# MeowMeowLady/InstanceSeg-Without-Voxelwise-Labeling

Hardware: AMD Instinct MI355X
Metric: voxels/sec end-to-end infer_simple (128^3 vol); 3D-conv TFLOPS vs roofline (higher is better)
Workload: dtype f32; 1 GPU; detection-mode infer_simple, host to host: pinned raw u16 volumes -> H2D -> norm1 -> dsn_body -> RPN -> proposals -> RoIAlign3D -> 2-MLP head -> decode -> NMS -> cross-tile NMS -> one all_gather of detections -> D2H; batch of 4 x (1x128^3) per rank, 3 distinct batches rotating [configs[2]]; volumes_per_rank=4

## Files before the change

include/m3d.h:

```cpp
#ifndef M3D_H_
#define M3D_H_
#include <stddef.h>
#include <stdint.h>

#ifdef __cplusplus
extern "C" {
#endif

#define M3D_OK 0
#define M3D_EINVAL (-1)
#define M3D_ELAUNCH (-2)
#define M3D_EWORKSPACE (-3)
#define M3D_EUNSUPPORTED (-4)

int m3d_version(void);
const char* m3d_error_string(int code);
const char* m3d_last_hip_error(void);
int m3d_set_option(const char* name, int value);
int m3d_get_option(const char* name, int* value);
int m3d_tuning_build(void);

int m3d_roi_align3d_forward(int aligned_slices, int aligned_height, int aligned_width, float spatial_scale,
                            int sampling_ratio, const float* d_features, int batch, int channels, int slices,
                            int height, int width, const float* d_rois, int num_rois, int roi_cols,
// ... 320 lines not shown
int m3d_conv3d_x3_pack(const float* d_weight, int cin, int cout, int relu_weights, void* d_packed, void* stream);
int m3d_conv3d_x3_forward(const float* d_x, const void* d_packed, float* d_out, int batch, int cin, int cout, int depth, int height,
                          int width, const float* d_in_offset, void* stream);
size_t m3d_conv3d_x3_workspace_bytes(int batch, int cin, int cout, int depth, int height, int width);
int m3d_conv3d_x3_forward_ws(const float* d_x, const void* d_packed, float* d_out, int batch, int cin, int cout, int depth, int height,
                             int width, const float* d_in_offset, void* d_workspace, size_t workspace_bytes, void* stream);
size_t m3d_conv3d_x3f_packed_bytes(int cin, int cout);
int m3d_conv3d_x3f_pack(const float* d_weight, int cin, int cout, int relu_weights, void* d_packed, void* stream);
int m3d_conv3d_x3f_forward_ws(const float* d_x, const void* d_packed, float* d_out, int batch, int cin, int cout, int depth, int height,
                              int width, const float* d_in_offset, const float* d_in_max, void* d_workspace, size_t workspace_bytes,
                              void* stream);
long long m3d_conv3d_x3_launch_units(int batch, int cin, int cout, int depth, int height, int width);

int m3d_conv3d_zw_supported(int cin, int cout, int depth, int height, int width, int pool);
size_t m3d_conv3d_zw_packed_bytes(int cin, int cout);
int m3d_conv3d_zw_pack(const float* d_weight, int cin, int cout, void* d_packed, void* stream);
int m3d_conv3d_zw_pack_dgrad(const float* d_weight, int cin, int cout, void* d_packed, void* stream);
int m3d_conv3d_zw_slots(void);
long long m3d_conv3d_zw_launch_units(int batch, int cin, int cout, int depth, int height, int width);
int m3d_conv3d_zw_bound_of(const float* d_x, long long n, float* d_slots, void* stream);
int m3d_conv3d_zw_forward(const float* d_in, const void* d_packed, float* d_out, int batch, int cin, int cout, int depth, int height,
                          int width, const float* d_scale, const float* d_shift, int relu, int pool, const float* d_in_max,
                          float* d_out_max, void* stream);
int m3d_conv3d_zn_supported(int cin, int cout, int depth, int height, int width);
size_t m3d_conv3d_zn_packed_bytes(int cin, int cout);
int m3d_conv3d_zn_pack(const float* d_weight, int cin, int cout, void* d_packed, void* stream);
int m3d_conv3d_zn_pack_dgrad(const float* d_weight, int cin, int cout, void* d_packed, void* stream);
long long m3d_conv3d_zn_launch_units(int batch, int cin, int cout, int depth, int height, int width);
int m3d_conv3d_zn_forward(const float* d_in, const void* d_packed, float* d_out, int batch, int cin, int cout, int depth, int height,
                          int width, const float* d_scale, const float* d_shift, int relu, const float* d_in_max, float* d_out_max,
                          void* stream);
int m3d_conv3d_zn_dilated_supported(int cin, int cout, int depth, int height, int width, int dilation);
long long m3d_conv3d_zn_dilated_launch_units(int batch, int cin, int cout, int depth, int height, int width, int dilation);
int m3d_conv3d_zn_dilated_forward(const float* d_in, const void* d_packed, float* d_out, int batch, int cin, int cout, int depth,
                                  int height, int width, int dilation, const float* d_scale, const float* d_shift, int relu,
                                  const float* d_in_max, float* d_out_max, void* stream);
int m3d_prm_strip_absmax(const float* d_strip, long long rows, int L, int pitch, int num_peaks, float* d_out, void* stream);
int m3d_conv3d_zw_forward_strip(const float* d_in, const void* d_packed, float* d_out, int cin, int cout, int depth, int height,
                                int width, const float* d_col_bound, int num_peaks, int pitch, void* stream);
int m3d_prm_strip_dgrad_prepare_zw(const float* d_gn, const void* d_packed, int cin, int cout, int num_peaks, int window, int in_slab,
                                   const int32_t* d_origin, const float* d_xnext, const float* d_norm, const float* d_scale,
                                   const float* d_up_offset, int depth, int height, int width, int out_slab,
                                   const float* d_col_bound, float* d_out, int32_t* d_origin_out, void* stream);

int m3d_prm_strip_dgrad_prepare(const float* d_gn, const float* d_packed, int cin, int cout, int num_peaks, int window, int in_slab,
                                const int32_t* d_origin, const float* d_xnext, const float* d_norm, const float* d_scale,
// ... 203 lines not shown
```

instanceseg-without-voxelwise-labeling_amd/csrc/fc_gemm.hip:

```cpp
#include <type_traits>

#include "f16x2.h"

namespace {

using namespace m3d::f16x2;

constexpr int BM = 128, BN = 128, BK = 32, LS = BK + 4;
constexpr int kStageFloats = (BM + BN) * LS;

struct FcArgs {
  const float* x; const float* w; const float* bias; float* out; float* part;
  int M, N, K, mt, nt, slices, chunks, relu;
  int slices_tail;
  int mt_full;
  int full_per_xcd, tail_per_xcd;
};

__global__ __launch_bounds__(256, 2) void fc_gemm_kernel(FcArgs a) {
  extern __shared__ float lds[];
  const int tid = threadIdx.x, lane = tid & 63, wave = tid >> 6;
  const int xcd = blockIdx.x & 7, idx = blockIdx.x >> 3;
  const int tiles_full = a.mt_full * a.nt, nfull = tiles_full * a.slices, ntail = (a.mt - a.mt_full) * a.nt * a.slices_tail;
  int slice, tile;
// ... 876 lines not shown
  }
  if (const int ts = m3d::opt(m3d::OPT_TUNE_FC_SLICES); ts > 0) bs = bt = ts < p.chunks ? ts : p.chunks;
  if (const int ts = m3d::opt(m3d::OPT_TUNE_FC_SLICES_TAIL); ts > 0) bt = ts < p.chunks ? ts : p.chunks;
  p.slices = bs; p.slices_tail = ntail_tiles ? bt : 1;
  p.full_per_xcd = (p.mt_full * p.nt * bs + 7) / 8;
  p.tail_per_xcd = (ntail_tiles * p.slices_tail + 7) / 8;
  return p;
}

X3Plan x3b_plan(int M, int N, int K) {
  X3Plan p{8, (M + 255) / 256, (N + 255) / 256, x3b_slices(M, N, K), 0};
  p.per_xcd = (p.mt * p.nt * p.slices + 7) / 8;
  return p;
}

inline bool f16x2_big_tiles(int M, int N) {
  const int w = m3d::opt(m3d::OPT_TUNE_FC_X3_ROWS);
  if (w == 128 || w == 256) return false;
  if (w == 512) return true;
  return M >= 384 && N >= 256;
}
X3Plan f16x2_plan(int M, int N, int K) { return f16x2_big_tiles(M, N) ? x3b_plan(M, N, K) : x3_plan(M, N, K); }

}

M3D_API int m3d_linear_plan(int kind, int M, int N, int K, int* tile_rows, int* tile_cols, int* slices, int* slices_tail,
                            int* full_row_tiles) {
  if (kind < 0 || kind > 3 || M <= 0 || N <= 0 || K <= 0) return M3D_EINVAL;
  if (K % (kind == 0 ? 4 : 32) != 0) return M3D_EUNSUPPORTED;
  int tr, tc, s, st, fm;
  if (kind == 0) {
    const Plan p = make_plan(M, N, K);
    tr = BM; tc = BN; s = p.slices; st = p.slices_tail; fm = p.mt_full;
  } else {
    const X3Plan p = kind == 1 ? x3_plan(M, N, K) : (kind == 2 ? x3b_plan(M, N, K) : f16x2_plan(M, N, K));
    tr = p.wr == 8 ? 256 : 64 * p.wr; tc = p.wr == 8 ? 256 : BN; s = st = p.slices; fm = p.mt;
  }
  if (tile_rows) *tile_rows = tr;
  if (tile_cols) *tile_cols = tc;
  if (slices) *slices = s;
  if (slices_tail) *slices_tail = st;
  if (full_row_tiles) *full_row_tiles = fm;
  return M3D_OK;
}

M3D_API size_t m3d_linear_workspace_bytes(int M, int N, int K) {
  if (M <= 0 || N <= 0 || K <= 0) return 0;
  const Plan p = make_plan(M, N, K);
  const int sm = p.slices > p.slices_tail ? p.slices : p.slices_tail;
  return sm > 1 ? (size_t)sm * M * N * sizeof(float) : 16;
}

M3D_API int m3d_linear_forward(const float* d_x, const float* d_weight, const float* d_bias, float* d_out, int M, int N, int K,
                               int relu, void* d_ws, size_t ws_bytes, void* stream) {
  if (M < 0 || N <= 0 || K <= 0) return M3D_EINVAL;
  if (M == 0) return M3D_OK;
  if (!d_x || !d_weight || !d_out) return M3D_EINVAL;
  if (K % 4 != 0 || ((uintptr_t)d_x & 15) || ((uintptr_t)d_weight & 15)) return M3D_EUNSUPPORTED;
  const Plan p = make_plan(M, N, K);
  const int sm = p.slices > p.slices_tail ? p.slices : p.slices_tail;
  if (sm > 1 && (!d_ws || ws_bytes < (size_t)sm * M * N * sizeof(float))) return M3D_EWORKSPACE;
  FcArgs a{d_x, d_weight, d_bias, d_out, (float*)d_ws, M, N, K, p.mt, p.nt, p.slices, p.chunks, relu, p.slices_tail, p.mt_full,
           p.full_per_xcd, p.tail_per_xcd};
  const size_t lds = sizeof(float) * 2 * kStageFloats;
  hipStream_t st = m3d::as_stream(stream);
  (void)hipFuncSetAttribute(reinterpret_cast<const void*>(fc_gemm_kernel), hipFuncAttributeMaxDynamicSharedMemorySize, (int)lds);
  hipLaunchKernelGGL(fc_gemm_kernel, dim3(8 * (p.full_per_xcd + p.tail_per_xcd)), dim3(256), lds, st, a);
  if (sm > 1) {
    const long long MN = (long long)M * N;
    long long blocks = (MN + 255) / 256;
    if (blocks > 4096) blocks = 4096;
    hipLaunchKernelGGL(fc_reduce_kernel, dim3((unsigned)blocks), dim3(256), 0, st, (const float*)d_ws, d_bias, d_out, MN, N, p.slices,
                       p.slices_tail, (long long)(p.mt_full < p.mt ? p.mt_full * BM : M) * N, relu, (unsigned*)nullptr);
  }
  return m3d::check_launch("linear_forward");
}

M3D_API size_t m3d_linear_bf16x3_packed_bytes(int N, int K) {
  if (N <= 0 || K <= 0 || K % 32 != 0) return 0;
  return (size_t)((N + BN - 1) / BN) * (K / 32) * X3_CHUNK_U4 * 16;
}
// ... 213 lines not shown
```

instanceseg-without-voxelwise-labeling_amd/m3d/_lib.py:

```python
import ctypes as C
import os

_HERE = os.path.dirname(os.path.abspath(__file__))
LIB_PATH = os.environ.get("M3D_LIB_PATH") or os.path.join(os.path.dirname(_HERE), "csrc", "libm3d.so")

M3D_OK = 0
_lib = None

SYMBOLS = [
    "m3d_version", "m3d_error_string", "m3d_last_hip_error", "m3d_set_option", "m3d_get_option", "m3d_tuning_build",
    "m3d_conv3d_stem5_prepare_dgrad_weights", "m3d_conv3d_stem5_dgrad", "m3d_norm1_workspace_bytes", "m3d_norm1", "m3d_norm1_batched", "m3d_norm1_stats",
    "m3d_linear_workspace_bytes", "m3d_linear_forward", "m3d_linear_bf16x3_packed_bytes", "m3d_linear_bf16x3_pack", "m3d_absmax", "m3d_linear_f16x2_packed_bytes", "m3d_linear_f16x2_pack", "m3d_linear_f16x2_workspace_bytes", "m3d_linear_f16x2_forward", "m3d_linear_f16x2_forward_bounds", "m3d_linear_plan",
    "m3d_box_head_workspace_bytes", "m3d_box_head_forward",
    "m3d_linear_bf16x3_workspace_bytes", "m3d_linear_bf16x3_forward", "m3d_mask_paste3d_workspace_bytes", "m3d_mask_paste3d", "m3d_linear_bf16x3_w32_workspace_bytes", "m3d_linear_bf16x3_w32_forward", "m3d_roi_align3d_tap_tables", "m3d_linear_bf16x3_roi_workspace_bytes", "m3d_linear_bf16x3_roi_forward",
    "m3d_fused_max_boxes", "m3d_compact_rows", "m3d_compact_rows2", "m3d_box_head_outputs", "m3d_conv3d_forward_split_sigmoid", "m3d_generate_proposals3d_batched_workspace_bytes", "m3d_generate_proposals3d_batched",
    "m3d_box_results3d_batched_workspace_bytes", "m3d_box_results3d_batched", "m3d_nms3d_batched_workspace_bytes", "m3d_nms3d_batched",
    "m3d_roi_align3d_forward", "m3d_roi_align3d_forward_exact", "m3d_roi_align3d_backward", "m3d_roi_align3d_workspace_bytes", "m3d_roi_align3d_forward_ws", "m3d_roi_align3d_forward_ws2", "m3d_roi_align3d_forward_ws3",
    "m3d_roi_align3d_backward_ordered_workspace_bytes", "m3d_roi_align3d_backward_ordered",
    "m3d_nms3d_workspace_bytes", "m3d_nms3d", "m3d_bbox_overlaps3d", "m3d_bbox_transform3d",
    "m3d_generate_proposals3d_workspace_bytes", "m3d_generate_proposals3d",
    "m3d_conv3d_packed_weight_bytes", "m3d_conv3d_pack_weights", "m3d_conv3d_forward", "m3d_conv3d_forward_dilated", "m3d_conv3d_forward_windowed", "m3d_conv3d_forward_pool2", "m3d_conv3d_direct_plan", "m3d_conv3d_direct_plan_count",
    "m3d_prm_seed", "m3d_prm_seed_ex", "m3d_prm_strip_geometry", "m3d_prm_prepare_plan", "m3d_prm_stem_dgrad_plan", "m3d_prm_select_peaks", "m3d_prm_select_peaks_ex", "m3d_prm_prepare", "m3d_prm_stem_prepare_weights", "m3d_prm_stem_dgrad", "m3d_prm_scatter", "m3d_prm_den_pool", "m3d_prm_stem_mfma_prepare_weights", "m3d_prm_stem_dgrad_fused_supported", "m3d_prm_stem_dgrad_fused", "m3d_prm_stem_dgrad_fused_ex", "m3d_prm_prepare_ex", "m3d_prm_stem_dgrad_fused_ex2", "m3d_prm_prepare_ex2", "m3d_prm_prepare_ex3", "m3d_prm_strip_dgrad_prepare", "m3d_conv3d_x3_packed_bytes", "m3d_conv3d_x3f_packed_bytes", "m3d_conv3d_x3f_pack", "m3d_conv3d_x3f_forward_ws", "m3d_reduce_minmax_multi", "m3d_reduce_minmax_multi_workspace_bytes", "m3d_conv3d_x3_supported", "m3d_conv3d_x3_pack", "m3d_conv3d_x3_forward", "m3d_conv3d_x3_workspace_bytes", "m3d_conv3d_x3_forward_ws", "m3d_conv3d_x3_launch_units", "m3d_conv3d_zw_supported", "m3d_conv3d_zw_packed_bytes", "m3d_conv3d_zw_pack", "m3d_conv3d_zw_slots", "m3d_conv3d_zw_launch_units", "m3d_conv3d_zw_bound_of", "m3d_conv3d_zw_forward", "m3d_conv3d_zw_forward_strip", "m3d_prm_strip_dgrad_prepare_zw", "m3d_prm_strip_absmax", "m3d_prm_small_dgrad_packed_bytes", "m3d_prm_small_dgrad_pack", "m3d_prm_small_dgrad_f16_supported", "m3d_prm_small_dgrad_f16_packed_bytes", "m3d_prm_small_dgrad_f16_pack", "m3d_prm_small_dgrad_f16_workspace_bytes", "m3d_prm_small_dgrad_f16", "m3d_prm_small_dgrad",
    "m3d_maxpool3d_2x_forward", "m3d_maxpool3d_2x_backward",
    "m3d_reduce_min_workspace_bytes", "m3d_reduce_min", "m3d_reduce_min_multi_workspace_bytes", "m3d_reduce_min_multi",
# ... 9 lines not shown
    "m3d_label_components_workspace_bytes", "m3d_label_components", "m3d_label_counts", "m3d_paint_spheres_workspace_bytes", "m3d_paint_spheres",
    "m3d_rpn_targets_workspace_bytes", "m3d_rpn_targets", "m3d_rpn_targets_wide", "m3d_rpn_loss",
    "m3d_box_head_targets_workspace_bytes", "m3d_box_head_targets", "m3d_box_head_target_blobs", "m3d_box_head_loss",
    "m3d_bn_stats", "m3d_bn_invstd", "m3d_bn_apply", "m3d_bn_backward",
    "m3d_sgd_chunk", "m3d_sgd_step", "m3d_sgd_step_scaled", "m3d_adam_step", "m3d_grad_clip_coef",
    "m3d_train_sample",
    "m3d_linear_dgrad_workspace_bytes", "m3d_linear_dgrad", "m3d_linear_wgrad_workspace_bytes", "m3d_linear_wgrad",
    "m3d_mask_targets", "m3d_mask_loss_workspace_bytes", "m3d_mask_loss",
    "m3d_conv3d_zw_pack_dgrad", "m3d_conv3d_gy_reduce",
    "m3d_peak_stimulation3d_workspace_bytes", "m3d_peak_stimulation3d", "m3d_peak_stimulation3d_backward",
    "m3d_upconv3d_2x_forward", "m3d_upconv3d_2x_dgrad_workspace_bytes", "m3d_upconv3d_2x_dgrad", "m3d_upconv3d_2x_wgrad_workspace_bytes",
    "m3d_upconv3d_2x_wgrad", "m3d_upconv3d_2x_slices",
    "m3d_conv3d_wgrad_dilated_workspace_bytes", "m3d_conv3d_wgrad_dilated", "m3d_conv3d_wgrad_dilated_tile", "m3d_conv3d_wgrad_dilated_plan",
    "m3d_conv3d_wgrad_narrow_supported", "m3d_conv3d_wgrad_narrow_workspace_bytes", "m3d_conv3d_wgrad_narrow_plan", "m3d_conv3d_wgrad_narrow",
    "m3d_conv3d_wgrad_narrow_f16x2_supported", "m3d_conv3d_wgrad_narrow_f16x2_workspace_bytes", "m3d_conv3d_wgrad_narrow_f16x2_plan",
    "m3d_conv3d_wgrad_narrow_f16x2",
    "m3d_conv3d_wgrad_narrow_dilated_f16x2_supported", "m3d_conv3d_wgrad_narrow_dilated_f16x2_workspace_bytes",
    "m3d_conv3d_wgrad_narrow_dilated_f16x2_plan", "m3d_conv3d_wgrad_narrow_dilated_f16x2",
    "m3d_conv3d_zn_supported", "m3d_conv3d_zn_packed_bytes", "m3d_conv3d_zn_pack", "m3d_conv3d_zn_pack_dgrad", "m3d_conv3d_zn_launch_units",
    "m3d_conv3d_zn_forward",
    "m3d_conv3d_zn_dilated_supported", "m3d_conv3d_zn_dilated_launch_units", "m3d_conv3d_zn_dilated_forward",
    "m3d_upconv3d_2x_f16x2_supported", "m3d_upconv3d_2x_f16x2_packed_bytes", "m3d_upconv3d_2x_f16x2_pack", "m3d_upconv3d_2x_forward_f16x2",
    "m3d_mask_tail_f16x2",
    "m3d_linear_backward_f16x2_supported", "m3d_linear_dgrad_f16x2_plan", "m3d_linear_wgrad_f16x2_plan",
    "m3d_linear_dgrad_f16x2_workspace_bytes", "m3d_linear_wgrad_f16x2_workspace_bytes", "m3d_linear_dgrad_f16x2", "m3d_linear_wgrad_f16x2",
]


class SgdTensor(C.Structure):
    _fields_ = [("p", C.c_void_p), ("g", C.c_void_p), ("m", C.c_void_p), ("n", C.c_longlong), ("lr", C.c_float), ("wd", C.c_float)]


class AdamTensor(C.Structure):
    _fields_ = [("p", C.c_void_p), ("g", C.c_void_p), ("m", C.c_void_p), ("v", C.c_void_p), ("n", C.c_longlong), ("lr_step", C.c_float),
                ("bc2_sqrt", C.c_float), ("wd", C.c_float)]


class GradTensor(C.Structure):
    _fields_ = [("g", C.c_void_p), ("n", C.c_longlong)]


class TrainImage(C.Structure):
    _fields_ = [("vol", C.c_void_p), ("stats", C.c_void_p), ("boxes", C.c_void_p), ("dtype", C.c_int), ("depth", C.c_int),
                ("height", C.c_int), ("width", C.c_int), ("num_boxes", C.c_int), ("start_max", C.c_int * 3)]


# ... 30 lines not shown
        raise M3DError("%s not built: run `python -c 'import __graft_entry__ as g; g.build()'` "
                       "or `make -C instanceseg-without-voxelwise-labeling_amd/csrc`. There is no CPU fallback." % path)
    L = C.CDLL(path)
    L.m3d_error_string.restype = C.c_char_p
    L.m3d_last_hip_error.restype = C.c_char_p
    L.m3d_conv3d_wino2_score.restype = C.c_double
    L.m3d_conv3d_wino2_local_score.restype = C.c_double
    L.m3d_prm_strip_geometry.restype = C.c_int64
    L.m3d_conv3d_x3_launch_units.restype = C.c_longlong
    L.m3d_conv3d_zw_launch_units.restype = C.c_longlong
    L.m3d_conv3d_zn_launch_units.restype = C.c_longlong
    L.m3d_conv3d_zn_dilated_launch_units.restype = C.c_longlong
    for n in ("m3d_roi_align3d_workspace_bytes", "m3d_roi_align3d_backward_ordered_workspace_bytes","m3d_nms3d_workspace_bytes", "m3d_generate_proposals3d_workspace_bytes",
              "m3d_conv3d_packed_weight_bytes", "m3d_conv3d_x3_packed_bytes", "m3d_conv3d_x3f_packed_bytes", "m3d_conv3d_zw_packed_bytes", "m3d_reduce_minmax_multi_workspace_bytes", "m3d_conv3d_x3_workspace_bytes", "m3d_reduce_min_workspace_bytes", "m3d_reduce_min_multi_workspace_bytes", "m3d_norm1_workspace_bytes", "m3d_prm_small_dgrad_packed_bytes", "m3d_prm_small_dgrad_f16_packed_bytes", "m3d_prm_small_dgrad_f16_workspace_bytes", "m3d_linear_workspace_bytes", "m3d_linear_bf16x3_packed_bytes", "m3d_linear_bf16x3_workspace_bytes", "m3d_linear_f16x2_packed_bytes", "m3d_linear_f16x2_workspace_bytes", "m3d_linear_bf16x3_w32_workspace_bytes", "m3d_linear_bf16x3_roi_workspace_bytes", "m3d_mask_paste3d_workspace_bytes", "m3d_generate_proposals3d_batched_workspace_bytes",
              "m3d_box_results3d_batched_workspace_bytes", "m3d_nms3d_batched_workspace_bytes", "m3d_otsu2d_workspace_bytes",
              "m3d_cc_workspace_bytes", "m3d_conv3d_wgrad_workspace_bytes", "m3d_conv3d_wino_packed_weight_bytes", "m3d_conv3d_wino2_packed_weight_bytes", "m3d_conv3d_wino2_workspace_bytes", "m3d_conv3d_wino2_local_workspace_bytes", "m3d_conv3d_stem_wino_packed_weight_bytes",
              "m3d_label_overlap_workspace_bytes", "m3d_box_union_overlap_workspace_bytes", "m3d_label_components_workspace_bytes",
              "m3d_paint_spheres_workspace_bytes", "m3d_rpn_targets_workspace_bytes", "m3d_box_head_targets_workspace_bytes",
              "m3d_box_head_workspace_bytes", "m3d_linear_dgrad_workspace_bytes", "m3d_linear_wgrad_workspace_bytes",
              "m3d_mask_loss_workspace_bytes", "m3d_conv3d_wgrad_f16x2_workspace_bytes", "m3d_peak_stimulation3d_workspace_bytes",
              "m3d_upconv3d_2x_dgrad_workspace_bytes", "m3d_upconv3d_2x_wgrad_workspace_bytes",
              "m3d_conv3d_wgrad_dilated_workspace_bytes", "m3d_conv3d_wgrad_narrow_workspace_bytes", "m3d_conv3d_zn_packed_bytes",
              "m3d_conv3d_wgrad_narrow_f16x2_workspace_bytes", "m3d_conv3d_wgrad_narrow_dilated_f16x2_workspace_bytes",
              "m3d_upconv3d_2x_f16x2_packed_bytes", "m3d_linear_dgrad_f16x2_workspace_bytes", "m3d_linear_wgrad_f16x2_workspace_bytes"):
        getattr(L, n).restype = C.c_size_t
    return L


def lib():
    global _lib
    if _lib is None:
        knobs = [(env, name) for env, name in _TUNE_ENV if env in os.environ]
        if knobs and "M3D_LIB_PATH" not in os.environ:
            _lib = _load(TUNE_LIB_PATH)
        else:
            _lib = _load(LIB_PATH)
        if knobs and _lib.m3d_tuning_build():
            for env, name in knobs:
                set_option(name, int(os.environ[env]))
    return _lib


class tuning:

    def __enter__(self):
        global _lib, _tune
        lib()
# ... 34 lines not shown
```

instanceseg-without-voxelwise-labeling_amd/m3d/model.py:

```python
import ctypes as C
import os

import numpy as np
import torch

from . import ops
from .conv_plan import LayerConv

BN_EPS = 1e-5


def dsn_layers(stride):
    if stride == 8:
        return [("conv1a", "bn1a", True), ("conv2a", "bn2a", False), ("conv2b", "bn2b", True), ("conv3a", "bn3a", False),
                ("conv3b", "bn3b", True), ("conv4a", "bn4a", False), ("conv4b", "bn4b", False)]
    return [("conv1a", "bn1a", True), ("conv2a", "bn2a", False), ("conv2b", "bn2b", True), ("conv3a", "bn3a", False),
            ("conv3b", "bn3b", False)]


class Probe:

    def __init__(self):
        self.spans = {}

# ... 38 lines not shown
class DetectorM3D:
    def __init__(self, params, cfg):
        self.cfg = cfg
        self.P = params
        self.probe = None
        n_head_convs = self._check_conv_head(params, cfg) if "Box_Head.convs.0.weight" in params else 0
        self.anchors = np.ascontiguousarray(cfg.anchors, dtype=np.float64)
        self.wino_mode = int(os.environ.get("M3D_WINO", "2"))
        self.use_wino = self.wino_mode != 0
        self.conv_f16 = self.use_wino and os.environ.get("M3D_CONV_F16", "1") == "1"
        self.head_conv_f16 = self.conv_f16 and os.environ.get("M3D_HEAD_CONV_F16", "0") == "1"
        self.body, self.convs = [], []
        for cname, bname, pool in dsn_layers(cfg.stride):
            c, b = "Conv_Body." + cname, "Conv_Body." + bname
            scale = (params[b + ".weight"] / torch.sqrt(params[b + ".running_var"] + BN_EPS)).contiguous()
            shift = ((params[c + ".bias"] - params[b + ".running_mean"]) * scale + params[b + ".bias"]).contiguous()
            self.convs.append(LayerConv(params[c + ".weight"], scale, shift, pool, self.wino_mode, self.conv_f16))
            self.body.append((self.convs[-1].conv, scale, shift, pool))
        self.rpn_conv_bias = params["RPN.RPN_conv.bias"].contiguous()
        self.rpn_conv = LayerConv(params["RPN.RPN_conv.weight"], None, self.rpn_conv_bias, False, self.wino_mode, self.conv_f16)
        self.A = params["RPN.RPN_cls_score.weight"].shape[0]
        w = torch.cat([params["RPN.RPN_cls_score.weight"], params["RPN.RPN_bbox_pred.weight"]], 0).contiguous()
        self.rpn_heads = ops.PackedConv3d(w)
        self.rpn_heads_bias = torch.cat([params["RPN.RPN_cls_score.bias"], params["RPN.RPN_bbox_pred.bias"]]).contiguous()
        self.conv_head = "Box_Head.convs.0.weight" in params
        self.has_head = self.conv_head or "Box_Head.fc1.weight" in params
        self.roi_gemm = os.environ.get("M3D_ROI_GEMM", "0") == "1"
        if self.has_head:
            self.outs_w = torch.cat([params["Box_Outs.cls_score.weight"], params["Box_Outs.bbox_pred.weight"]], 0).contiguous()
            self.outs_b = torch.cat([params["Box_Outs.cls_score.bias"], params["Box_Outs.bbox_pred.bias"]]).contiguous()
            self.fc_split = {}
            mode = os.environ.get("M3D_FC_SPLIT", "f16x2")
            if self.conv_head:
                self.head_convs = self._conv_head_layers(params, n_head_convs)
            if mode != "0":
                cls = ops.SplitLinear if mode in ("bf16x3", "1") else ops.SplitLinearF16
                for name in (("fc",) if self.conv_head else ("fc1", "fc2")):
                    w = params["Box_Head.%s.weight" % name]
                    if cls.supported(w):
                        self.fc_split[name] = cls(w, params["Box_Head.%s.bias" % name])

    @staticmethod
    def _check_conv_head(params, cfg):
        n = 0
        while "Box_Head.convs.%d.weight" % (2 * n) in params:
            n += 1
# ... 18 lines not shown
        kw = dict(narrow_f16=True) if self.head_conv_f16 else {}
        return [LayerConv(params["Box_Head.convs.%d.weight" % (2 * i)], None, params["Box_Head.convs.%d.bias" % (2 * i)].contiguous(), False,
                          self.wino_mode, self.conv_f16, **kw) for i in range(n)]

    def body_layer(self, li, x, bound_slot=None):
        return self.convs[li](x, self._bound, bound_slot)

    @staticmethod
    def _carried_bound(x):
        b = getattr(x, "_m3d_bound", None)
        return b[0] if b is not None and b[1] == x._version else None

    @staticmethod
    def _bound(x):
        b = DetectorM3D._carried_bound(x)
        return b if b is not None else ops.ZwConv3d.bound_of(x)

    def span(self, name):
        return self.probe(name) if self.probe is not None else _NOSPAN

    ISSUED_FRACTION = {"winograd F(2x2,3x3)": 4.0 / 9.0, "winograd F(2x4,3x3)": 1.0 / 3.0, "winograd F(2,3)x": 2.0 / 3.0,
                       "winograd F(2,5)x stem": 78.0 / 125.0, "direct": 1.0, "f16x2 F(2,3)z": 2.0}
    F16_KINDS = ("f16x2 F(2,3)z",)

    def conv_work(self, batch, size):
        out = {}
        S, H, W = size

        def record(layer):
            kind = layer.plan((batch, S, H, W)).kind
            f16 = kind in self.F16_KINDS
            pad = (layer.cout + 63) // 64 * 64 / float(layer.cout) if f16 else (layer.cout + 31) // 32 * 32 / float(layer.cout)
            alg = 2.0 * layer.cin * layer.cout * layer.k ** 3 * S * H * W * batch
            return dict(algorithmic_flop=alg, issued_flop=alg * self.ISSUED_FRACTION[kind] * pad, kernel=kind,
                        shape="%d->%d k%d @ %dx%dx%d" % (layer.cin, layer.cout, layer.k, S, H, W), dtype="f16" if f16 else "f32")
        for (cname, _, pool), layer in zip(dsn_layers(self.cfg.stride), self.convs):
            out[cname] = record(layer)
            if pool:
                S, H, W = S // 2, H // 2, W // 2
        r = record(self.rpn_conv)
        cout, nh = self.rpn_conv.cout, 7 * self.A
        alg_h = 2.0 * cout * nh * S * H * W * batch
        out["rpn"] = dict(algorithmic_flop=r["algorithmic_flop"] + alg_h, issued_flop=r["issued_flop"] + alg_h * ((nh + 31) // 32 * 32 / float(nh)),
                          dtype=r["dtype"], kernel=r["kernel"] + " (3^3 conv) + direct (the two 1^3 heads as one conv)",
                          shape="%d->%d k3, %d->%d k1 @ %dx%dx%d" % (self.rpn_conv.cin, cout, cout, nh, S, H, W))
        return out

    def conv_body(self, x, first=0, last=None):
        names = dsn_layers(self.cfg.stride)
        slots = torch.zeros((len(self.body) + 1, ops.ZwConv3d.SLOTS), dtype=torch.float32, device=x.device) if self.conv_f16 else None
        for li in range(first, len(self.body) if last is None else last):
            with self.span(names[li][0]):
                x = self.body_layer(li, x, slots[li] if slots is not None else None)
        if slots is not None:
            x._m3d_head_bound = slots[len(self.body)]
        return x

    def capture_body(self, x, first=0, last=None):
        torch.cuda.synchronize()
        side = torch.cuda.Stream()
        side.wait_stream(torch.cuda.current_stream())
        with torch.cuda.stream(side):
            for _ in range(2):
                self.conv_body(x, first, last)
        torch.cuda.current_stream().wait_stream(side)
        g = torch.cuda.CUDAGraph()
        with torch.cuda.graph(g):
            out = self.conv_body(x, first, last)
        return g.replay, out

    def rpn(self, feat):
        return self.rpn_outputs(self.rpn_conv(feat, self._bound, out_max=False))

    def rpn_outputs(self, h):
        return self.rpn_heads.split_sigmoid(h, self.A, shift=self.rpn_heads_bias)

    def _fused_ok(self, prob):
        total = prob.shape[-4] * prob.shape[-3] * prob.shape[-2] * prob.shape[-1]
        k = total if (self.cfg.pre_nms_topN <= 0 or self.cfg.pre_nms_topN >= total) else self.cfg.pre_nms_topN
        return k <= ops.fused_max_boxes()

    def proposals(self, prob, deltas, im_info, item=0):
        c = self.cfg
        if self._fused_ok(prob):
            rois, probs, kidx, num = ops.generate_proposals3d_batched(
                prob[item:item + 1], deltas[item:item + 1], self.anchors, float(c.stride), im_info, c.pre_nms_topN,
                c.post_nms_topN, c.rpn_nms_thresh, c.rpn_min_size, first_batch_index=item)
            r = int(num.item())
            return rois[0, :r], probs[0, :r].unsqueeze(1), kidx[0, :r]
        return ops.generate_proposals3d(prob[item].contiguous(), deltas[item], self.anchors, float(c.stride), im_info,
                                        c.pre_nms_topN, c.post_nms_topN, c.rpn_nms_thresh, c.rpn_min_size, batch_index=item)

    def box_head_outputs(self, feat, rois, clip_to=None):
        c, P = self.cfg, self.P
        if self.conv_head:
            return self._conv_head_outputs(feat, rois, clip_to)
        if self.probe is None and self._one_call_ok(feat, rois, int(rois.shape[0])):
# ... 277 lines not shown
```

instanceseg-without-voxelwise-labeling_amd/m3d/ops.py:

```python
import ctypes as C
import math
import threading

import numpy as np
import torch

from ._lib import lib, check, M3DError, SgdTensor, AdamTensor, GradTensor, BoxHead, TrainImage, MaskImage

BBOX_XFORM_CLIP = float(np.log(1000. / 16.))

__all__ = ["compact_rows", "compact_rows2", "box_head_outputs", "roi_align3d_forward", "roi_align3d_backward", "roi_align3d_backward_ordered", "nms3d", "bbox_overlaps3d", "bbox_transform3d",
           "generate_proposals3d", "generate_proposals3d_batched", "box_results3d_batched", "nms3d_batched", "fused_max_boxes", "PackedConv3d", "maxpool3d_2x", "maxpool3d_2x_backward", "reduce_min", "reduce_min_multi", "norm1", "norm1_batched", "norm1_stats", "train_sample", "linear", "linear_plan", "linear_dgrad", "linear_wgrad", "linear_dgrad_f16x2", "linear_wgrad_f16x2", "linear_backward_f16x2_supported", "linear_dgrad_f16x2_plan", "linear_wgrad_f16x2_plan", "upconv3d_2x_forward", "upconv3d_2x_dgrad", "upconv3d_2x_wgrad", "upconv3d_2x_slices", "UPCONV_KINDS", "UpConvF16", "SplitLinear", "linear_roi_fused", "mask_paste3d",
           "otsu2d_batch", "prm_quantize_u8", "prm_quantize_windows_u8", "prm_quantize_windows_compact_u8", "roi_normalize", "conv3d_wgrad", "conv3d_wgrad_f16x2", "conv3d_wgrad_f16x2_supported", "conv3d_wgrad_f16x2_plan", "conv3d_wgrad_narrow_f16x2", "conv3d_wgrad_narrow_f16x2_supported", "conv3d_wgrad_narrow_f16x2_plan", "conv3d_direct_plan", "conv3d_bias_grad", "conv3d_gy_reduce", "WinoConv3d", "ZwConv3d", "ZnConv3d", "X3Conv3d", "StemWinoConv3d", "gaussian_filter_u16", "median_filter3_u16", "cc_largest_batch", "binary_closing6_batch", "paint_instances", "paint_instances_into", "paint_finish", "paint_begin", "crop_offsets", "upload_packed", "conv3d_windowed", "prm_seed", "strip_geometry", "prm_prepare_plan", "prm_stem_dgrad_plan", "PRM_PREPARE_KERNELS", "PRM_STEM_DGRAD_LAYOUTS", "prm_select_peaks", "PinnedPool", "upload", "prm_prepare", "prm_stem_dgrad", "prm_stem_prepare_weights", "SmallWindowDgrad", "prm_den_pool", "prm_stem_mfma_weights", "prm_stem_dgrad_fused", "prm_stem_dgrad_fused_supported", "prm_scatter", "conv3d_stem5_dgrad", "conv3d_stem5_dgrad_weights", "label_overlap", "label_iou_best", "box_union_overlap_counts", "Overlap", "IouBest", "LABEL_LIMIT", "label_components", "label_counts", "paint_spheres", "rpn_target_sets", "rpn_target_blobs", "rpn_loss_grad", "box_head_target_sets", "box_head_target_blobs", "box_head_loss_grad", "mask_target_sets", "mask_loss_grad", "bn_stats", "bn_invstd", "bn_apply", "bn_backward", "sgd_step", "sgd_chunk", "sgd_step_scaled", "adam_step", "grad_clip_coef", "M3DError", "BBOX_XFORM_CLIP", "W_PLAIN", "W_RELU", "W_DGRAD", "W_DGRAD_RELU"]

W_PLAIN, W_RELU, W_DGRAD, W_DGRAD_RELU = 0, 1, 2, 3


def _stream():
    return C.c_void_p(torch.cuda.current_stream().cuda_stream)


def _need_gpu(*ts):
    for t in ts:
        if t is not None and not t.is_cuda:
# ... 1600 lines not shown
    def units(self, shape, dilation=1):
        if int(dilation) == 1:
            return super().units(shape)
        B = int(shape[0]) if len(shape) == 5 else 1
        D, H, W = (int(v) for v in shape[-3:])
        return int(lib().m3d_conv3d_zn_dilated_launch_units(B, self.cin, self.cout, D, H, W, int(dilation)))

    def __call__(self, x, in_max, scale=None, shift=None, relu=False, out=None, out_max=None, dilation=1):
        x, out, out_max = self._operands(x, in_max, out, out_max)
        B, cin, D, H, W = x.shape
        if int(dilation) != 1:
            check(lib().m3d_conv3d_zn_dilated_forward(_ptr(x), _ptr(self.packed), _ptr(out), B, cin, self.cout, D, H, W, int(dilation),
                                                      _ptr(scale) if scale is not None else None, _ptr(shift) if shift is not None else None,
                                                      int(bool(relu)), _ptr(in_max), _ptr(out_max) if out_max is not None else None,
                                                      _stream()), "conv3d_zn_dilated_forward")
            return out, out_max
        check(lib().m3d_conv3d_zn_forward(_ptr(x), _ptr(self.packed), _ptr(out), B, cin, self.cout, D, H, W,
                                          _ptr(scale) if scale is not None else None, _ptr(shift) if shift is not None else None,
                                          int(bool(relu)), _ptr(in_max), _ptr(out_max) if out_max is not None else None,
                                          _stream()), "conv3d_zn_forward")
        return out, out_max


class WinoConv3d(object):

    def __init__(self, weight, two_d=False, local=False):
        _need_gpu(weight)
        w = _f32c(weight)
        assert w.dim() == 5 and tuple(w.shape[2:]) == (3, 3, 3)
        self.cout, self.cin = int(w.shape[0]), int(w.shape[1])
        self.two_d = bool(two_d)
        self.local = bool(local) and self.two_d
        L = lib()
        self._bytes, self._pack, self._fwd, self._pool = \
            (L.m3d_conv3d_wino2_packed_weight_bytes, L.m3d_conv3d_wino2_pack_weights, L.m3d_conv3d_wino2_forward,
             L.m3d_conv3d_wino2_forward_pool2) if self.two_d else \
            (L.m3d_conv3d_wino_packed_weight_bytes, L.m3d_conv3d_wino_pack_weights, L.m3d_conv3d_wino_forward,
             L.m3d_conv3d_wino_forward_pool2)
        nbytes = self._bytes(self.cin, self.cout)
        self.packed = torch.empty((nbytes // 4,), dtype=torch.float32, device=w.device)
        check(self._pack(_ptr(w), self.cin, self.cout, _ptr(self.packed), _stream()), "wino_pack")

    def supports(self, width, shape=None):
        if width < (12 if self.two_d else 24):
            return False
        if self.two_d and shape is not None:
# ... 993 lines not shown
```

Before: 2.954 billion voxels/s.

## Add f16x2 MFMA pointwise RPN head kernel and small-N linear path

Adds a split-f16 MFMA 1x1x1 convolution kernel for the fused RPN cls/bbox heads, with sigmoid applied to the first split channels, and wires it behind an opt-in environment flag. It also routes linear layers with N<=32 to a new per-wave dot-product kernel instead of the tiled GEMM. The head path is meant to replace the direct FP32 pointwise conv with matrix-core work. The small-N path is meant to avoid large GEMM tiles that are mostly wasted when N is tiny. The f16 path is off by default (M3D_RPN_HEADS_F16=0), so only the small-N linear change runs by default.

After: 2.954 billion voxels/s, median of 2. No clear change (-0.0%).

```diff
diff --git a/include/m3d.h b/include/m3d.h
--- a/include/m3d.h
+++ b/include/m3d.h
@@ -366,6 +366,12 @@
 int m3d_conv3d_zw_forward(const float* d_in, const void* d_packed, float* d_out, int batch, int cin, int cout, int depth, int height,
                           int width, const float* d_scale, const float* d_shift, int relu, int pool, const float* d_in_max,
                           float* d_out_max, void* stream);
+int m3d_conv1x1_f16x2_supported(int cin, int cout);
+size_t m3d_conv1x1_f16x2_packed_bytes(int cin, int cout);
+int m3d_conv1x1_f16x2_pack(const float* d_weight, int cin, int cout, void* d_packed, void* stream);
+int m3d_conv1x1_f16x2_split_sigmoid(const float* d_in, const void* d_packed, float* d_out_sigmoid, float* d_out_rest, int batch, int cin,
+                                    int cout, int split, int depth, int height, int width, const float* d_shift, const float* d_in_max,
+                                    void* stream);
 int m3d_conv3d_zn_supported(int cin, int cout, int depth, int height, int width);
 size_t m3d_conv3d_zn_packed_bytes(int cin, int cout);
 int m3d_conv3d_zn_pack(const float* d_weight, int cin, int cout, void* d_packed, void* stream);
diff --git a/instanceseg-without-voxelwise-labeling_amd/csrc/conv1x1_f16.hip b/instanceseg-without-voxelwise-labeling_amd/csrc/conv1x1_f16.hip
--- /dev/null
+++ b/instanceseg-without-voxelwise-labeling_amd/csrc/conv1x1_f16.hip
@@ -0,0 +1,189 @@
+#include "f16x2.h"
+
+namespace {
+
+using namespace m3d::f16x2;
+
+constexpr int PW_NT = 512, PW_WAVES = 8;
+constexpr int PW_TV = 32;
+constexpr int PW_CG = 32 * PW_WAVES;
+constexpr int PW_STEP_UNITS = PW_WAVES * 128;
+constexpr int PW_PF = 4;
+constexpr int PW_MAX_CIN = 1024;
+
+__global__ __launch_bounds__(256) void pw_pack_kernel(const float* __restrict__ w, int cin, int cout, u32x4* __restrict__ packed,
+                                                      const float* __restrict__ wamax) {
+  float sw, inv;
+  f16_scale_of(*wamax, sw, inv);
+  const int steps = cin / 16, ncg = (cout + PW_CG - 1) / PW_CG;
+  const long long total = (long long)ncg * steps * PW_WAVES * 64;
+  for (long long e = (long long)blockIdx.x * 256 + threadIdx.x; e < total; e += (long long)gridDim.x * 256) {
+    const int row = (int)(e & 31), kh = (int)((e >> 5) & 1), cb = (int)((e >> 6) & (PW_WAVES - 1));
+    const long long r = e >> 9;
+    const int t = (int)(r % steps), cg = (int)(r / steps);
+    const int co = cg * PW_CG + cb * 32 + row;
+    u32x4 ph, pl;
+#pragma unroll
+    for (int j = 0; j < 4; ++j) {
+      f16x2 hh, ll;
+#pragma unroll
+      for (int u = 0; u < 2; ++u) {
+        const float v = co < cout ? w[(size_t)co * cin + t * 16 + 8 * kh + 2 * j + u] * sw : 0.f;
+        cut(v, hh, ll, u);
+      }
+      ph[j] = __builtin_bit_cast(unsigned, hh); pl[j] = __builtin_bit_cast(unsigned, ll);
+    }
+    u32x4* dst = packed + ((size_t)(cg * steps + t) * PW_WAVES + cb) * 128 + kh * 32 + row;
+    dst[0] = ph; dst[64] = pl;
+  }
+}
+
+struct PwArgs {
+  const float* x; const u32x4* wp; const float* wamax; const float* bias; const float* in_max;
+  float* out_sig; float* out_rest;
+  int cin, cout, split;
+  long long V;
+};
+
+__global__ __launch_bounds__(PW_NT, 4) void conv1x1_f16_kernel(PwArgs a) {
+  extern __shared__ float lds_f[];
+  u32x4* const lds = reinterpret_cast<u32x4*>(lds_f);
+  const int tid = threadIdx.x, lane = tid & 63;
+  const int wave = __builtin_amdgcn_readfirstlane(tid >> 6);
+  const int b = blockIdx.y, cg = blockIdx.z;
+  const long long v0 = (long long)blockIdx.x * PW_TV;
+  const int steps = a.cin / 16, kgs = a.cin / 8, plane = kgs * PW_TV;
+
+  float xs, inv_x, inv_w;
+  {
+    float sw_;
+    f16_scale_of(bound_of_slots(a.in_max, lane), xs, inv_x);
+    f16_scale_of(*a.wamax, sw_, inv_w);
+  }
+
+  const int co0 = cg * PW_CG + wave * 32;
+  const bool active = co0 < a.cout;
+  const u32x4* wq = a.wp + ((size_t)cg * steps * PW_WAVES + wave) * 128 + lane;
+  f16x8 nh[PW_PF], nl[PW_PF];
+  auto load_w = [&](int g) __attribute__((always_inline)) {
+#pragma unroll
+    for (int i = 0; i < PW_PF; ++i) {
+      const int t = min(g * PW_PF + i, steps - 1);
+      nh[i] = __builtin_bit_cast(f16x8, wq[(size_t)t * PW_STEP_UNITS]);
+      nl[i] = __builtin_bit_cast(f16x8, wq[(size_t)t * PW_STEP_UNITS + 64]);
+    }
+  };
+  if (active) load_w(0);
+
+  const float* xb = a.x + (size_t)b * a.cin * a.V;
+  for (int it0 = 0; it0 < plane; it0 += 2 * PW_NT) {
+    float v[2][8];
+    int it[2];
+#pragma unroll
+    for (int i = 0; i < 2; ++i) {
+      it[i] = it0 + i * PW_NT + tid;
+      const int itc = min(it[i], plane - 1);
+      const int kg = itc >> 5, vox = itc & 31;
+      const long long p = min(v0 + vox, a.V - 1);
+      const float* src = xb + (size_t)(8 * kg) * a.V + p;
+#pragma unroll
+      for (int j = 0; j < 8; ++j) v[i][j] = src[(size_t)j * a.V];
+    }
+#pragma unroll
+    for (int i = 0; i < 2; ++i) {
+      if (it[i] >= plane) continue;
+      u32x4 ph, pl;
+#pragma unroll
+      for (int j = 0; j < 4; ++j) {
+        f16x2 hh, ll;
+        cut(v[i][2 * j] * xs, v[i][2 * j + 1] * xs, hh, ll);
+        ph[j] = __builtin_bit_cast(unsigned, hh); pl[j] = __builtin_bit_cast(unsigned, ll);
+      }
+      lds[it[i]] = ph;
+      lds[plane + it[i]] = pl;
+    }
+  }
+  __syncthreads();
+  if (!active) return;
+
+  const int c = lane & 31, h = lane >> 5;
+  f32x16 acc[2];
+#pragma unroll
+  for (int i = 0; i < 2; ++i)
+#pragma unroll
+    for (int g = 0; g < 16; ++g) acc[i][g] = 0.f;
+  const int groups = (steps + PW_PF - 1) / PW_PF;
+  for (int g = 0; g < groups; ++g) {
+    f16x8 ch[PW_PF], cl[PW_PF];
+#pragma unroll
+    for (int i = 0; i < PW_PF; ++i) { ch[i] = nh[i]; cl[i] = nl[i]; }
+    if (g + 1 < groups) load_w(g + 1);
+#pragma unroll
+    for (int i = 0; i < PW_PF; ++i) {
+      const int t = g * PW_PF + i;
+      if (t < steps) {
+        const f16x8 bh = __builtin_bit_cast(f16x8, lds[(2 * t + h) * PW_TV + c]);
+        const f16x8 bl = __builtin_bit_cast(f16x8, lds[plane + (2 * t + h) * PW_TV + c]);
+        mfma3(ch[i], cl[i], bh, bl, acc[i & 1]);
+      }
+    }
+  }
+
+  const long long p = v0 + c;
+  if (p >= a.V) return;
+  const float un = inv_x * inv_w;
+  const int nrest = a.cout - a.split;
+#pragma unroll
+  for (int g = 0; g < 16; ++g) {
+    const int co = co0 + acc_row(g) + 4 * h;
+    if (co >= a.cout) continue;
+    float v = (acc[0][g] + acc[1][g]) * un;
+    if (a.bias) v += a.bias[co];
+    if (co < a.split) a.out_sig[((size_t)b * a.split + co) * a.V + p] = m3d::sigmoid_f32(v);
+    else a.out_rest[((size_t)b * nrest + (co - a.split)) * a.V + p] = v;
+  }
+}
+
+inline size_t pw_plane_bytes(int cin, int cout) { return (size_t)((cout + PW_CG - 1) / PW_CG) * (cin / 16) * PW_STEP_UNITS * 16; }
+
+}
+
+M3D_API int m3d_conv1x1_f16x2_supported(int cin, int cout) {
+  return cin >= 16 && cin % 16 == 0 && cin <= PW_MAX_CIN && cout >= 1 && (cout + PW_CG - 1) / PW_CG <= 65535;
+}
+
+M3D_API size_t m3d_conv1x1_f16x2_packed_bytes(int cin, int cout) {
+  if (!m3d_conv1x1_f16x2_supported(cin, cout)) return 0;
+  return pw_plane_bytes(cin, cout) + 256;
+}
+
+M3D_API int m3d_conv1x1_f16x2_pack(const float* d_weight, int cin, int cout, void* d_packed, void* stream) {
+  if (!d_weight || !d_packed || cin <= 0 || cout <= 0) return M3D_EINVAL;
+  if (!m3d_conv1x1_f16x2_supported(cin, cout) || ((uintptr_t)d_packed & 15)) return M3D_EUNSUPPORTED;
+  float* wamax = reinterpret_cast<float*>(static_cast<char*>(d_packed) + pw_plane_bytes(cin, cout));
+  if (const int rc = m3d_absmax(d_weight, (long long)cout * cin, wamax, stream)) return rc;
+  hipLaunchKernelGGL(pw_pack_kernel, dim3(256), dim3(256), 0, m3d::as_stream(stream), d_weight, cin, cout, (u32x4*)d_packed, (const float*)wamax);
+  return m3d::check_launch("conv1x1_f16x2_pack");
+}
+
+M3D_API int m3d_conv1x1_f16x2_split_sigmoid(const float* d_in, const void* d_packed, float* d_out_sigmoid, float* d_out_rest, int batch,
+                                            int cin, int cout, int split, int depth, int height, int width, const float* d_shift,
+                                            const float* d_in_max, void* stream) {
+  if (!d_in || !d_packed || !d_out_sigmoid || !d_out_rest || !d_in_max || batch <= 0 || depth <= 0 || height <= 0 || width <= 0)
+    return M3D_EINVAL;
+  if (split <= 0 || split >= cout) return M3D_EINVAL;
+  if (!m3d_conv1x1_f16x2_supported(cin, cout) || batch > 65535) return M3D_EUNSUPPORTED;
+  PwArgs a{};
+  a.x = d_in; a.wp = static_cast<const u32x4*>(d_packed); a.bias = d_shift; a.in_max = d_in_max;
+  a.wamax = reinterpret_cast<const float*>(static_cast<const char*>(d_packed) + pw_plane_bytes(cin, cout));
+  a.out_sig = d_out_sigmoid; a.out_rest = d_out_rest;
+  a.cin = cin; a.cout = cout; a.split = split;
+  a.V = (long long)depth * height * width;
+  const long long tiles = (a.V + PW_TV - 1) / PW_TV;
+  if (tiles > 0x7FFFFFFFll) return M3D_EUNSUPPORTED;
+  const size_t lds = (size_t)cin * PW_TV * 4;
+  (void)hipFuncSetAttribute(reinterpret_cast<const void*>(conv1x1_f16_kernel), hipFuncAttributeMaxDynamicSharedMemorySize, (int)lds);
+  hipLaunchKernelGGL(conv1x1_f16_kernel, dim3((unsigned)tiles, (unsigned)batch, (unsigned)((cout + PW_CG - 1) / PW_CG)), dim3(PW_NT), lds,
+                     m3d::as_stream(stream), a);
+  return m3d::check_launch("conv1x1_f16x2_split_sigmoid");
+}
diff --git a/instanceseg-without-voxelwise-labeling_amd/csrc/fc_gemm.hip b/instanceseg-without-voxelwise-labeling_amd/csrc/fc_gemm.hip
--- a/instanceseg-without-voxelwise-labeling_amd/csrc/fc_gemm.hip
+++ b/instanceseg-without-voxelwise-labeling_amd/csrc/fc_gemm.hip
@@ -922,6 +922,54 @@
 }
 X3Plan f16x2_plan(int M, int N, int K) { return f16x2_big_tiles(M, N) ? x3b_plan(M, N, K) : x3_plan(M, N, K); }
 
+constexpr int kSmallN = 32;
+constexpr int SN_ROWS = 2, SN_WAVES = 4;
+
+template <int NN>
+__global__ __launch_bounds__(64 * SN_WAVES) void fc_small_n_kernel(const float* __restrict__ x, const float* __restrict__ w,
+                                                                   const float* __restrict__ bias, float* __restrict__ out, int M, int N,
+                                                                   int K, int relu) {
+  const int lane = threadIdx.x & 63, wave = threadIdx.x >> 6;
+  const int m0 = (blockIdx.x * SN_WAVES + wave) * SN_ROWS;
+  if (m0 >= M) return;
+  const float* px[SN_ROWS];
+#pragma unroll
+  for (int r = 0; r < SN_ROWS; ++r) px[r] = x + (size_t)min(m0 + r, M - 1) * K;
+  float acc[SN_ROWS][NN];
+#pragma unroll
+  for (int r = 0; r < SN_ROWS; ++r)
+#pragma unroll
+    for (int n = 0; n < NN; ++n) acc[r][n] = 0.f;
+  for (int k = 4 * lane; k < K; k += 256) {
+    f32x4 vx[SN_ROWS];
+#pragma unroll
+    for (int r = 0; r < SN_ROWS; ++r) vx[r] = *reinterpret_cast<const f32x4*>(px[r] + k);
+#pragma unroll
+    for (int n = 0; n < NN; ++n) {
+      const f32x4 vw = *reinterpret_cast<const f32x4*>(w + (size_t)min(n, N - 1) * K + k);
+#pragma unroll
+      for (int r = 0; r < SN_ROWS; ++r)
+#pragma unroll
+        for (int j = 0; j < 4; ++j) acc[r][n] = fmaf(vx[r][j], vw[j], acc[r][n]);
+    }
+  }
+#pragma unroll
+  for (int r = 0; r < SN_ROWS; ++r) {
+    float mine = 0.f;
+#pragma unroll
+    for (int n = 0; n < NN; ++n) {
+      float v = acc[r][n];
+#pragma unroll
+      for (int o = 32; o >= 1; o >>= 1) v += __shfl_xor(v, o);
+      if (lane == n) mine = v;
+    }
+    if (lane < N && m0 + r < M) {
+      if (bias) mine += bias[lane];
+      out[(size_t)(m0 + r) * N + lane] = relu ? fmaxf(mine, 0.f) : mine;
+    }
+  }
+}
+
 }
 
 M3D_API int m3d_linear_plan(int kind, int M, int N, int K, int* tile_rows, int* tile_cols, int* slices, int* slices_tail,
@@ -957,6 +1005,12 @@
   if (M == 0) return M3D_OK;
   if (!d_x || !d_weight || !d_out) return M3D_EINVAL;
   if (K % 4 != 0 || ((uintptr_t)d_x & 15) || ((uintptr_t)d_weight & 15)) return M3D_EUNSUPPORTED;
+  if (N <= kSmallN) {
+    const unsigned grid = (unsigned)((M + SN_ROWS * SN_WAVES - 1) / (SN_ROWS * SN_WAVES));
+    auto kern = N <= 4 ? fc_small_n_kernel<4> : (N <= 16 ? fc_small_n_kernel<16> : fc_small_n_kernel<32>);
+    hipLaunchKernelGGL(kern, dim3(grid), dim3(64 * SN_WAVES), 0, m3d::as_stream(stream), d_x, d_weight, d_bias, d_out, M, N, K, relu);
+    return m3d::check_launch("linear_forward");
+  }
   const Plan p = make_plan(M, N, K);
   const int sm = p.slices > p.slices_tail ? p.slices : p.slices_tail;
   if (sm > 1 && (!d_ws || ws_bytes < (size_t)sm * M * N * sizeof(float))) return M3D_EWORKSPACE;
diff --git a/instanceseg-without-voxelwise-labeling_amd/m3d/_lib.py b/instanceseg-without-voxelwise-labeling_amd/m3d/_lib.py
--- a/instanceseg-without-voxelwise-labeling_amd/m3d/_lib.py
+++ b/instanceseg-without-voxelwise-labeling_amd/m3d/_lib.py
@@ -55,6 +55,7 @@
     "m3d_conv3d_zn_dilated_supported", "m3d_conv3d_zn_dilated_launch_units", "m3d_conv3d_zn_dilated_forward",
     "m3d_upconv3d_2x_f16x2_supported", "m3d_upconv3d_2x_f16x2_packed_bytes", "m3d_upconv3d_2x_f16x2_pack", "m3d_upconv3d_2x_forward_f16x2",
     "m3d_mask_tail_f16x2",
+    "m3d_conv1x1_f16x2_supported", "m3d_conv1x1_f16x2_packed_bytes", "m3d_conv1x1_f16x2_pack", "m3d_conv1x1_f16x2_split_sigmoid",
     "m3d_linear_backward_f16x2_supported", "m3d_linear_dgrad_f16x2_plan", "m3d_linear_wgrad_f16x2_plan",
     "m3d_linear_dgrad_f16x2_workspace_bytes", "m3d_linear_wgrad_f16x2_workspace_bytes", "m3d_linear_dgrad_f16x2", "m3d_linear_wgrad_f16x2",
 ]
@@ -131,7 +132,7 @@
               "m3d_upconv3d_2x_dgrad_workspace_bytes", "m3d_upconv3d_2x_wgrad_workspace_bytes",
               "m3d_conv3d_wgrad_dilated_workspace_bytes", "m3d_conv3d_wgrad_narrow_workspace_bytes", "m3d_conv3d_zn_packed_bytes",
               "m3d_conv3d_wgrad_narrow_f16x2_workspace_bytes", "m3d_conv3d_wgrad_narrow_dilated_f16x2_workspace_bytes",
-              "m3d_upconv3d_2x_f16x2_packed_bytes", "m3d_linear_dgrad_f16x2_workspace_bytes", "m3d_linear_wgrad_f16x2_workspace_bytes"):
+              "m3d_upconv3d_2x_f16x2_packed_bytes", "m3d_conv1x1_f16x2_packed_bytes", "m3d_linear_dgrad_f16x2_workspace_bytes", "m3d_linear_wgrad_f16x2_workspace_bytes"):
         getattr(L, n).restype = C.c_size_t
     return L
 
diff --git a/instanceseg-without-voxelwise-labeling_amd/m3d/model.py b/instanceseg-without-voxelwise-labeling_amd/m3d/model.py
--- a/instanceseg-without-voxelwise-labeling_amd/m3d/model.py
+++ b/instanceseg-without-voxelwise-labeling_amd/m3d/model.py
@@ -84,6 +84,8 @@
         self.A = params["RPN.RPN_cls_score.weight"].shape[0]
         w = torch.cat([params["RPN.RPN_cls_score.weight"], params["RPN.RPN_bbox_pred.weight"]], 0).contiguous()
         self.rpn_heads = ops.PackedConv3d(w)
+        heads_f16 = self.conv_f16 and os.environ.get("M3D_RPN_HEADS_F16", "0") == "1" and ops.PointwiseF16.supported(w)
+        self.rpn_heads_f16 = ops.PointwiseF16(w) if heads_f16 else None
         self.rpn_heads_bias = torch.cat([params["RPN.RPN_cls_score.bias"], params["RPN.RPN_bbox_pred.bias"]]).contiguous()
         self.conv_head = "Box_Head.convs.0.weight" in params
         self.has_head = self.conv_head or "Box_Head.fc1.weight" in params
@@ -148,6 +150,7 @@
     ISSUED_FRACTION = {"winograd F(2x2,3x3)": 4.0 / 9.0, "winograd F(2x4,3x3)": 1.0 / 3.0, "winograd F(2,3)x": 2.0 / 3.0,
                        "winograd F(2,5)x stem": 78.0 / 125.0, "direct": 1.0, "f16x2 F(2,3)z": 2.0}
     F16_KINDS = ("f16x2 F(2,3)z",)
+    HEADS_F16_ISSUED = 3.0
 
     def conv_work(self, batch, size):
         out = {}
@@ -167,19 +170,25 @@
         r = record(self.rpn_conv)
         cout, nh = self.rpn_conv.cout, 7 * self.A
         alg_h = 2.0 * cout * nh * S * H * W * batch
-        out["rpn"] = dict(algorithmic_flop=r["algorithmic_flop"] + alg_h, issued_flop=r["issued_flop"] + alg_h * ((nh + 31) // 32 * 32 / float(nh)),
-                          dtype=r["dtype"], kernel=r["kernel"] + " (3^3 conv) + direct (the two 1^3 heads as one conv)",
+        heads_f16 = self.rpn_heads_f16 is not None and r["kernel"] in self.F16_KINDS
+        out["rpn"] = dict(algorithmic_flop=r["algorithmic_flop"] + alg_h,
+                          issued_flop=r["issued_flop"] + alg_h * ((nh + 31) // 32 * 32 / float(nh)) * (self.HEADS_F16_ISSUED if heads_f16 else 1.0),
+                          dtype=r["dtype"], kernel=r["kernel"] + " (3^3 conv) + " + ("f16x2 pointwise" if heads_f16 else "direct")
+                          + " (the two 1^3 heads as one conv)",
                           shape="%d->%d k3, %d->%d k1 @ %dx%dx%d" % (self.rpn_conv.cin, cout, cout, nh, S, H, W))
         return out
 
     def conv_body(self, x, first=0, last=None):
         names = dsn_layers(self.cfg.stride)
-        slots = torch.zeros((len(self.body) + 1, ops.ZwConv3d.SLOTS), dtype=torch.float32, device=x.device) if self.conv_f16 else None
+        rows = len(self.body) + (2 if self.rpn_heads_f16 is not None else 1)
+        slots = torch.zeros((rows, ops.ZwConv3d.SLOTS), dtype=torch.float32, device=x.device) if self.conv_f16 else None
         for li in range(first, len(self.body) if last is None else last):
             with self.span(names[li][0]):
                 x = self.body_layer(li, x, slots[li] if slots is not None else None)
         if slots is not None:
             x._m3d_head_bound = slots[len(self.body)]
+            if self.rpn_heads_f16 is not None:
+                x._m3d_rpn_bound = slots[len(self.body) + 1]
         return x
 
     def capture_body(self, x, first=0, last=None):
@@ -196,9 +205,14 @@
         return g.replay, out
 
     def rpn(self, feat):
-        return self.rpn_outputs(self.rpn_conv(feat, self._bound, out_max=False))
+        if self.rpn_heads_f16 is None:
+            return self.rpn_outputs(self.rpn_conv(feat, self._bound, out_max=False))
+        return self.rpn_outputs(self.rpn_conv(feat, self._bound, out_max=feat.__dict__.pop("_m3d_rpn_bound", None)))
 
     def rpn_outputs(self, h):
+        b = self._carried_bound(h) if self.rpn_heads_f16 is not None else None
+        if b is not None:
+            return self.rpn_heads_f16.split_sigmoid(h, self.A, b, shift=self.rpn_heads_bias)
         return self.rpn_heads.split_sigmoid(h, self.A, shift=self.rpn_heads_bias)
 
     def _fused_ok(self, prob):
diff --git a/instanceseg-without-voxelwise-labeling_amd/m3d/ops.py b/instanceseg-without-voxelwise-labeling_amd/m3d/ops.py
--- a/instanceseg-without-voxelwise-labeling_amd/m3d/ops.py
+++ b/instanceseg-without-voxelwise-labeling_amd/m3d/ops.py
@@ -1646,6 +1646,37 @@
         return out, out_max
 
 
+class PointwiseF16(object):
+
+    @staticmethod
+    def supported(weight):
+        if weight.dim() not in (2, 5) or any(int(v) != 1 for v in weight.shape[2:]):
+            return False
+        return bool(lib().m3d_conv1x1_f16x2_supported(int(weight.shape[1]), int(weight.shape[0])))
+
+    def __init__(self, weight):
+        _need_gpu(weight)
+        w = _f32c(weight)
+        assert self.supported(w)
+        self.cout, self.cin = int(w.shape[0]), int(w.shape[1])
+        nbytes = lib().m3d_conv1x1_f16x2_packed_bytes(self.cin, self.cout)
+        self.packed = torch.empty((nbytes,), dtype=torch.uint8, device=w.device)
+        check(lib().m3d_conv1x1_f16x2_pack(_ptr(w), self.cin, self.cout, _ptr(self.packed), _stream()), "conv1x1_f16x2_pack")
+
+    def split_sigmoid(self, x, split, in_max, shift=None):
+        _need_gpu(x, in_max)
+        x = _f32c(x)
+        B, Cin, D, H, W = x.shape
+        if Cin != self.cin:
+            raise ValueError("expected %d input channels, got %d" % (self.cin, Cin))
+        assert in_max.numel() == _F16x2Conv3d.SLOTS and in_max.dtype == torch.float32
+        a = torch.empty((B, split, D, H, W), dtype=torch.float32, device=x.device)
+        b = torch.empty((B, self.cout - split, D, H, W), dtype=torch.float32, device=x.device)
+        check(lib().m3d_conv1x1_f16x2_split_sigmoid(_ptr(x), _ptr(self.packed), _ptr(a), _ptr(b), B, Cin, self.cout, int(split), D, H, W,
+                                                    _ptr(shift), _ptr(in_max), _stream()), "conv1x1_f16x2_split_sigmoid")
+        return a, b
+
+
 class WinoConv3d(object):
 
     def __init__(self, weight, two_d=False, local=False):
```
